# gallilmaimon/DISSC

Hardware: AMD Instinct MI355X
Metric: audio-sec/sec (RTF) HiFi-GAN resynth, 10s x32 batch (higher is better)
Workload: dtype f32

## Files before the change

dissc_amd/_lib.py:

```python
import ctypes
import os

import torch

_HERE = os.path.dirname(os.path.abspath(__file__))
_LIB_NAME = "libdissc_hip.so"


def library_path():
    return os.environ.get("DISSC_HIP_LIB") or os.path.join(_HERE, _LIB_NAME)


class DisscError(RuntimeError):
    pass


class DisscTensor(ctypes.Structure):
    _fields_ = [("name", ctypes.c_char_p), ("data", ctypes.c_void_p),
                ("shape", ctypes.c_int64 * 4), ("ndim", ctypes.c_int32)]


MAX_UPS, MAX_RK = 8, 4


class DisscGenConfig(ctypes.Structure):
    _fields_ = [("model_in_dim", ctypes.c_int32), ("upsample_initial_channel", ctypes.c_int32),
                ("num_upsamples", ctypes.c_int32), ("upsample_rates", ctypes.c_int32 * MAX_UPS),
                ("upsample_kernel_sizes", ctypes.c_int32 * MAX_UPS), ("num_kernels", ctypes.c_int32),
                ("resblock_kernel_sizes", ctypes.c_int32 * MAX_RK),
                ("resblock_dilations", (ctypes.c_int32 * 3) * MAX_RK),
                ("num_embeddings", ctypes.c_int32), ("embedding_dim", ctypes.c_int32),
                ("num_speakers", ctypes.c_int32), ("has_f0", ctypes.c_int32), ("has_spkr", ctypes.c_int32)]


class DisscConvLaunch(ctypes.Structure):
    _fields_ = [(n, ctypes.c_int32) for n in ("family", "cfg", "bm", "bn", "rows", "p0", "np", "ntap", "pad_left")]


class DisscBf3Info(ctypes.Structure):
    _fields_ = [(n, ctypes.c_int32) for n in ("bm", "bn", "small_grid", "tile", "cols", "h4", "pad")]


class DisscWino8Plan(ctypes.Structure):
    _fields_ = [(n, ctypes.c_int32) for n in ("mi", "ni", "wps", "r", "ns", "unit", "ot", "cpr", "gx", "gy")]


def _load():
    path = library_path()
    if not os.path.exists(path):
        raise DisscError(
            f"{path} not found: build the HIP library first "
            "(python -c 'import __graft_entry__ as g; g.build()').  "
            "dissc_amd has no CPU fallback.")
    L = ctypes.CDLL(path)
    vp, i32, i64p = ctypes.c_void_p, ctypes.c_int, ctypes.c_void_p
    L.dissc_last_error.restype = ctypes.c_char_p
    L.dissc_abi_version.restype = i32
    L.dissc_device_count.restype = i32
    L.dissc_device_name.argtypes = [i32, ctypes.c_char_p, ctypes.c_size_t]
    L.dissc_gen_create.argtypes = [ctypes.POINTER(DisscGenConfig), ctypes.POINTER(DisscTensor),
                                   ctypes.c_size_t, ctypes.POINTER(vp)]
    L.dissc_gen_create_ex.argtypes = [ctypes.POINTER(DisscGenConfig), ctypes.POINTER(DisscTensor),
                                      ctypes.c_size_t, i32, ctypes.POINTER(vp)]
    L.dissc_gen_destroy.argtypes = [vp]
    L.dissc_gen_destroy.restype = None
    L.dissc_gen_hop.argtypes = [vp]
    L.dissc_gen_workspace_bytes.argtypes = [vp, i32, i32]
    L.dissc_gen_workspace_bytes.restype = ctypes.c_size_t
    L.dissc_gen_flops.argtypes = [vp, ctypes.c_int64]
    L.dissc_gen_flops.restype = ctypes.c_double
    L.dissc_gen_flops_executed.argtypes = [vp, ctypes.c_int64]
    L.dissc_gen_flops_executed.restype = ctypes.c_double
    L.dissc_gen_forward.argtypes = [vp, i64p, vp, i64p, vp, i32, i32, vp, vp, ctypes.c_size_t, vp]
    L.dissc_conv1d.argtypes = [vp, vp, vp, vp, vp, i32, i32, i32, i32, i32, i32, i32, i32,
                               ctypes.c_float, vp]
    L.dissc_conv_transpose1d.argtypes = [vp, vp, vp, vp, vp, i32, i32, i32, i32, i32, i32, i32, i32,
                                         ctypes.c_float, vp]
    L.dissc_conv1d_prec.argtypes = [vp, vp, vp, vp, vp, i32, i32, i32, i32, i32, i32, i32, i32, ctypes.c_float, i32, vp]
    L.dissc_conv_transpose1d_prec.argtypes = [vp, vp, vp, vp, vp, i32, i32, i32, i32, i32, i32, i32, i32, ctypes.c_float, i32, vp]
    L.dissc_pred_create.argtypes = [i32, ctypes.POINTER(DisscTensor), ctypes.c_size_t, ctypes.POINTER(vp)]
    L.dissc_pred_destroy.argtypes = [vp]
    L.dissc_pred_destroy.restype = None
    L.dissc_pred_workspace_bytes.argtypes = [vp, i32, i32]
    L.dissc_pred_workspace_bytes.restype = ctypes.c_size_t
    L.dissc_len_set_norm.argtypes = [vp, ctypes.c_float, ctypes.c_float]
    L.dissc_len_forward.argtypes = [vp, vp, vp, vp, i32, i32, vp, i32, vp, ctypes.c_size_t, vp]
    L.dissc_pitch_forward.argtypes = [vp, vp, vp, vp, i32, i32, i32, vp, vp, i32, vp, i32, vp,
                                      ctypes.c_size_t, vp]
    L.dissc_dedup.argtypes = [vp, vp, i32, i32, vp, vp, vp, vp]
    L.dissc_len_carryover.argtypes = [vp, vp, i32, i32, vp, vp, vp]
    L.dissc_expand.argtypes = [vp, vp, vp, i32, i32, vp, i32, vp]
    L.dissc_hubert_create.argtypes = [i32, ctypes.POINTER(DisscTensor), ctypes.c_size_t, vp, i32,
                                      ctypes.POINTER(vp)]
    L.dissc_hubert_create_ex.argtypes = [i32, ctypes.POINTER(DisscTensor), ctypes.c_size_t, vp, i32, i32,
                                         ctypes.POINTER(vp)]
    L.dissc_hubert_precision.argtypes = [vp]
    L.dissc_hubert_destroy.argtypes = [vp]
    L.dissc_hubert_destroy.restype = None
    L.dissc_hubert_frames.argtypes = [i32]
    L.dissc_hubert_workspace_bytes.argtypes = [vp, i32, i32]
    L.dissc_hubert_workspace_bytes.restype = ctypes.c_size_t
    L.dissc_hubert_forward.argtypes = [vp, vp, vp, i32, i32, vp, vp, vp, ctypes.c_size_t, vp]
    L.dissc_kmeans_assign.argtypes = [vp, vp, vp, i32, i32, i32, vp, vp]
    L.dissc_mfma_peak.argtypes = [i32, ctypes.POINTER(ctypes.c_float)]
    L.dissc_erf_check.argtypes = [vp, vp, i32, vp]
    L.dissc_attention.argtypes = [vp, vp, i32, i32, i32, i32, vp, vp]
    L.dissc_layernorm_cf.argtypes = [vp, vp, vp, vp, i32, i32, i32, ctypes.c_float, vp, vp]
    L.dissc_set_option.argtypes = [ctypes.c_char_p, i32]
    L.dissc_get_option.argtypes = [ctypes.c_char_p, ctypes.POINTER(ctypes.c_int)]
    L.dissc_conv_bench.argtypes = [i32] * 9 + [ctypes.POINTER(ctypes.c_float)]
    L.dissc_conv1d_s2.argtypes = [vp, vp, vp, vp, vp] + [i32] * 9 + [vp]
    L.dissc_conv1d_s2_prec.argtypes = [vp, vp, vp, vp, vp] + [i32] * 9 + [vp]
    L.dissc_linear_prec.argtypes = [vp, vp, vp, vp, vp, vp] + [i32] * 7 + [vp]
    L.dissc_conv_s2_bench.argtypes = [i32] * 5 + [ctypes.POINTER(ctypes.c_float)]
    L.dissc_pair_bench.argtypes = [i32] * 8 + [ctypes.POINTER(ctypes.c_float)]
    L.dissc_pair_info.argtypes = [i32] * 3 + [ctypes.POINTER(ctypes.c_int)] * 2
    L.dissc_conv_info.argtypes = [i32] * 7 + [ctypes.POINTER(DisscConvLaunch), i32, ctypes.POINTER(ctypes.c_int)]
    L.dissc_wino8_info.argtypes = [i32] * 6 + [ctypes.POINTER(DisscWino8Plan)]
    L.dissc_resblock1d_bf3.argtypes = [vp, vp, vp, vp, vp, i32, i32, i32, vp, i32, i32, ctypes.c_float, i32, ctypes.c_float, i32, i32, vp]
    L.dissc_bf3_info.argtypes = [i32] * 6 + [vp, i32, i32, ctypes.POINTER(DisscBf3Info)]
    L.dissc_respair1d.argtypes = [vp] * 8 + [i32] * 6 + [ctypes.c_float, i32, ctypes.c_float, i32, vp]
    L.dissc_wav_postprocess.argtypes = [vp, vp, i32, i32, vp]
    L.dissc_pitch_stats.argtypes = [vp, vp, i32, vp, vp, vp, vp]
    i64 = ctypes.c_longlong
    L.dissc_pack_rows.argtypes = [vp, i64, vp, vp, i32, i32, vp, vp]
    L.dissc_comm_unique_id.argtypes = [ctypes.c_char_p]
# ... 76 lines not shown
```

dissc_amd/csrc/common.h:

```cpp
#pragma once
#include <hip/hip_runtime.h>
#include <stdint.h>
#include <stdio.h>

#include <atomic>
#include <functional>
#include <mutex>
#include <string>
#include <vector>

#include "../../include/dissc_hip.h"

#ifndef DISSC_EXPERIMENTAL
#define DISSC_EXPERIMENTAL 0
#endif

namespace dissc {

void set_error(const char* fmt, ...);

#define DISSC_OPTION_LIST_DEFAULT(X) \
  X(multistream, 1, "multistream") \
  X(pair_dma, 1, "pair_dma") \
  X(precision, 0, "precision") \
  X(enc_precision, 0, "enc_precision") \
  X(use_mfma32, 1, "mfma32") \
  X(ragged_enum, 1, "ragged_enum") \
  X(lin128, 1, "lin128") \
  X(conv2s128, 1, "conv2s128") \
  X(xcd_order, 11, "xcd_order") \
  X(xcd_mg, 0, "xcd_mg") \
  X(small_grid, 1, "small_grid") \
  X(kernel_dbg, 0, "kernel_dbg") \
  X(wino_sv, 1, "wino_sv") \
  X(wino8_c64_wide, 3, "wino8_c64_wide") \
  X(wino8_mask, 0450770550, "wino8_mask") \
  X(wino8_r4_mask, 0770770010, "wino8_r4_mask") \
  X(wino8_r4, 1, "wino8_r4") \
  X(wino8, 1, "wino8") \
  X(wino, 1, "wino") \
  X(hubert_split, 1, "hubert_split") \
  X(pair_max_c, 32, "pair_max_c") \
  X(pair_f23, 3, "pair_f23") \
  X(pair_tc6, 3, "pair_tc6") \
  X(pair_f23_c64, 1, "pair_f23_c64") \
  X(pair_tc6_c64, 1, "pair_tc6_c64")
#define DISSC_OPTION_LIST_EXPERIMENTAL(X) \
  X(graphs, 0, "graphs") \
  X(graph_frames, 2048, "graph_frames") \
  X(enc_tc, 0, "enc_tc") \
  X(s2tc_xmode, 0, "s2tc_xmode") \
  X(pair_wino, 0, "pair_wino") \
  X(pairw_chv, 2, "pairw_chv")
#if DISSC_EXPERIMENTAL
#define DISSC_OPTION_LIST(X) DISSC_OPTION_LIST_DEFAULT(X) DISSC_OPTION_LIST_EXPERIMENTAL(X)
#else
#define DISSC_OPTION_LIST(X) DISSC_OPTION_LIST_DEFAULT(X)
#endif
struct Options {
#define DISSC_OPT_FIELD(f, d, k) int f = d;
  DISSC_OPTION_LIST(DISSC_OPT_FIELD)
#undef DISSC_OPT_FIELD
#if !DISSC_EXPERIMENTAL
#define DISSC_OPT_CONST(f, d, k) static constexpr int f = d;
  DISSC_OPTION_LIST_EXPERIMENTAL(DISSC_OPT_CONST)
#undef DISSC_OPT_CONST
#endif
  int cfg_for_bm[5] = {6, 5, 7, 1, 0};
  int cfg32_for_bm[4] = {3, 2, 1, 0};
};
extern Options g_defaults;
extern thread_local const Options* t_opts;
inline const Options& opts() { return t_opts ? *t_opts : g_defaults; }
extern int g_graph_hits, g_graph_captures;
struct OptScope {
  const Options* prev;
  explicit OptScope(const Options* o) : prev(t_opts) { t_opts = o; }
  ~OptScope() { t_opts = prev; }
  OptScope(const OptScope&) = delete;
  OptScope& operator=(const OptScope&) = delete;
};

extern thread_local int g_conv_prec;
struct PrecScope {
  const int prev;
  explicit PrecScope(int p) : prev(g_conv_prec) { g_conv_prec = p; }
  ~PrecScope() { g_conv_prec = prev; }
  PrecScope(const PrecScope&) = delete;
  PrecScope& operator=(const PrecScope&) = delete;
};

#define DISSC_HIP_CHECK(expr)                                                       \
  do {                                                                              \
    hipError_t _e = (expr);                                                         \
    if (_e != hipSuccess) {                                                         \
      dissc::set_error("%s failed: %s (%s:%d)", #expr, hipGetErrorString(_e),       \
                       __FILE__, __LINE__);                                         \
      return DISSC_EHIP;                                                            \
    }                                                                               \
// ... 222 lines not shown
struct DevPairW {
  float* w1 = nullptr;
  float* w2 = nullptr;
  float* b1 = nullptr;
  float* b2 = nullptr;
  int C = 0, KS = 0, dil = 1;
  int form = 0;
};
bool pair_f23_supported(int C, int KS, int dil);
bool pair_tc6_supported(int C, int KS, int dil);
bool pairw43_built();
int pack_pairw43(const float* w, int C, int KS, float** dev);
int launch_pairw43(const DevPairW& pw, const float* x, float* out, const Batch& bt, const EpiSpec& ep, int ld, float slope,
                   hipStream_t stream);
bool pairw_supported(int C, int KS, int dil);
bool pair_form_supported(int form, int C, int KS, int dil);
int pair_reg_tile(int form, int C, int KS, int dil);
int make_pairw(const float* w1, const float* b1, const float* w2, const float* b2, int C, int KS, int dil, int form, DevPairW& pw);
void free_pairw(DevPairW& pw);
int launch_respair_wino(const DevPairW& pw, const float* x, float* out, const Batch& bt, const EpiSpec& ep, int ld, float slope,
                        hipStream_t stream);

bool respair_supported(int C, int KS, int dil);
int launch_respair(const DevConv& c1, const DevConv& c2, const float* x, float* out, const Batch& bt, const EpiSpec& ep, int ld,
                   float slope, hipStream_t stream);

bool resblock_bf3_supported(int C, int KS, const int* dil);
void pack_resblock_bf3(int C, int KS, const float* const* w6, std::vector<float>& packed);
struct Bf3Block { int C, KS; const int* dil; const float *wpack, *bias; };
int launch_resblock_bf3(const Bf3Block& blk, const float* x, const Batch& bt, const EpiSpec& ep, int ld, float slope, int m0, int m1,
                        hipStream_t stream);
struct ResblockBf3Plan { int NW, NI, COLS, PAD, H4, BN; };
int resblock_bf3_plan(int C, int KS, const int* dil, int m0, int m1, ResblockBf3Plan& p);

struct DevS2tc {
  float* wpack = nullptr;
  float* bias = nullptr;
  int CIN = 0, M = 0, act = 0;
};
bool s2tc_supported(int Cout, int Cin, int KS, int stride);
int make_s2tc(const float* w, const float* bias, int Cout, int Cin, DevS2tc& dc);
void free_s2tc(DevS2tc& dc);
double s2tc_executed_macs_per_out(int Cout, int Cin);
int run_s2tc(const DevS2tc& dc, const float* x, float* out, const Batch& bt, int ldx, int ldo, hipStream_t stream);

struct ZeroSpans {
  float* p[DISSC_MAX_RK];
  int n;
};
void launch_embed_concat(const int64_t* code, const float* f0, const int64_t* spkr,
                         const float* dict_w, const float* spkr_w, const int32_t* lengths, int B,
                         int T, int E, int has_f0, int has_spkr, int n_codes, int n_spk, float* x,
                         int ldx, const ZeroSpans& zs, hipStream_t stream);
void launch_conv_post(const float* x, const float* w, const float* bias, const int32_t* lengths,
                      int len_mul, int B, int C, int KS, int L, int ldx, long long x_bstride,
                      float slope, float* wav, int ldw, hipStream_t stream);
void launch_wav_postprocess(float* wav, const int32_t* n_samples, int B, int ld,
                            hipStream_t stream);

}
```

dissc_amd/csrc/gen_misc.hip:

```cpp
#include "common.h"

namespace dissc {

__global__ void embed_concat_kernel(const int64_t* __restrict__ code, const float* __restrict__ f0,
                                    const int64_t* __restrict__ spkr,
                                    const float* __restrict__ dict_w,
                                    const float* __restrict__ spkr_w,
                                    const int32_t* __restrict__ lengths, int T, int E, int has_f0,
                                    int has_spkr, int n_codes, int n_spk, float* __restrict__ x,
                                    int ldx, int C, const ZeroSpans zs) {
  const int b = blockIdx.z;
  const int c = blockIdx.y;
  const int t = blockIdx.x * blockDim.x + threadIdx.x;
  if (blockIdx.x == 0 && c == 0 && b == 0 && threadIdx.x < ZERO_TAIL)
    for (int j = 0; j < zs.n; ++j) zs.p[j][threadIdx.x] = 0.f;
  const int len = lengths ? lengths[b] : T;
  if (t >= len) return;
  float v;
  if (c < E) {
    long long id = code[(size_t)b * T + t];
    id = id < 0 ? 0 : (id >= n_codes ? n_codes - 1 : id);
    v = dict_w[(size_t)id * E + c];
  } else if (has_f0 && c == E) {
    v = f0[(size_t)b * T + t];
  } else {
    long long id = spkr[b];
    id = id < 0 ? 0 : (id >= n_spk ? n_spk - 1 : id);
    v = spkr_w[(size_t)id * E + (c - E - (has_f0 ? 1 : 0))];
  }
  x[((size_t)b * C + c) * ldx + t] = v;
}

void launch_embed_concat(const int64_t* code, const float* f0, const int64_t* spkr,
                         const float* dict_w, const float* spkr_w, const int32_t* lengths, int B,
                         int T, int E, int has_f0, int has_spkr, int n_codes, int n_spk, float* x,
                         int ldx, const ZeroSpans& zs, hipStream_t stream) {
  const int C = E + (has_f0 ? 1 : 0) + (has_spkr ? E : 0);
  dim3 grid((T + 127) / 128, C, B);
  hipLaunchKernelGGL(embed_concat_kernel, grid, dim3(128), 0, stream, code, f0, spkr, dict_w,
                     spkr_w, lengths, T, E, has_f0, has_spkr, n_codes, n_spk, x, ldx, C, zs);
}

constexpr int POST_TILE = 512;
__global__ void __launch_bounds__(256) conv_post_kernel(const float* __restrict__ x,
                                                        const float* __restrict__ w,
                                                        const float* __restrict__ bias,
                                                        const int32_t* __restrict__ lengths,
                                                        int len_mul, int C, int KS, int L, int ldx,
                                                        long long x_bstride, float slope,
                                                        float* __restrict__ wav, int ldw) {
  extern __shared__ float xs[];
  const int b = blockIdx.y;
  const int len = lengths ? lengths[b] * len_mul : L;
  const int t0 = blockIdx.x * POST_TILE;
  float* wb = wav + (size_t)b * ldw;
  if (t0 >= len) {
    for (int i = threadIdx.x; i < POST_TILE; i += 256)
      if (t0 + i < L) wb[t0 + i] = 0.f;
    return;
  }
  const int halo = KS / 2;
  const int W = POST_TILE + KS - 1;
  const float* xb = x + (size_t)b * x_bstride;
  for (int e = threadIdx.x; e < C * W; e += 256) {
    const int ci = e / W, u = e - ci * W;
    const int t = t0 - halo + u;
    float v = 0.f;
    if (t >= 0 && t < len) {
      v = xb[(size_t)ci * ldx + t];
      v = v > 0.f ? v : v * slope;
    }
    xs[e] = v;
  }
  __syncthreads();
  const float bz = bias[0];
#pragma unroll
  for (int i = 0; i < POST_TILE / 256; ++i) {
    const int u = threadIdx.x + i * 256;
    const int t = t0 + u;
    if (t >= L) continue;
    float s = bz;
    for (int ci = 0; ci < C; ++ci)
      for (int j = 0; j < KS; ++j) s = fmaf(w[ci * KS + j], xs[ci * W + u + j], s);
    wb[t] = t < len ? tanhf(s) : 0.f;
  }
}

__global__ void __launch_bounds__(256) conv_post7_kernel(const float* __restrict__ x, const float* __restrict__ w,
                                                         const float* __restrict__ bias,
                                                         const int32_t* __restrict__ lengths, int len_mul, int C,
                                                         int L, int ldx, long long x_bstride, float slope,
                                                         float* __restrict__ wav, int ldw) {
  const int b = blockIdx.y;
// ... 221 lines not shown
```

dissc_amd/csrc/generator.hip:

```cpp
#include <algorithm>
#include <functional>
#include <map>
#include <mutex>
#include <string>
#include <tuple>
#include <vector>

#include "gen_plan.h"

using namespace dissc;


static hipStream_t shared_aux_stream(int chain, int prio) {
  static std::mutex mu;
  static std::map<std::tuple<int, int, int>, hipStream_t> pool;
  int dev = 0;
  if (hipGetDevice(&dev) != hipSuccess) return nullptr;
  std::lock_guard<std::mutex> lock(mu);
  auto key = std::make_tuple(dev, chain, prio);
  auto it = pool.find(key);
  if (it != pool.end()) return it->second;
  hipStream_t st = nullptr;
  if (hipStreamCreateWithPriority(&st, hipStreamNonBlocking, prio) != hipSuccess) return nullptr;
  pool[key] = st;
  return st;
}

struct dissc_gen {
  Options opt;
  DisscGenConfig cfg;
  int hop = 1;
  DevConv conv_pre;
  std::vector<std::vector<DevConv>> ups;
  std::vector<ChainPlan> plan;
  std::vector<DevConv> rb1, rb2;
  std::vector<DevPairW> pw;
  std::vector<float*> fused_w, fused_b;
  float* post_w = nullptr;
  float* post_b = nullptr;
  int post_C = 0, post_KS = 0;
  float* dict_w = nullptr;
  float* spkr_w = nullptr;
  std::vector<int> stage_C, stage_mul;
  hipStream_t aux[DISSC_MAX_RK] = {nullptr, nullptr, nullptr, nullptr};
  hipEvent_t ev_x = nullptr, ev_fin[DISSC_MAX_RK] = {nullptr, nullptr, nullptr, nullptr};
  struct GraphEntry {
    const void *code, *f0, *spkr, *lengths, *out, *ws;
    int B, T;
    hipGraphExec_t exec;
    unsigned long long stamp;
  };
  std::vector<GraphEntry> graphs;
  hipStream_t cap_stream = nullptr;
  unsigned long long graph_clock = 0;
  int graph_failures = 0;
  ~dissc_gen() {
    for (auto& e : graphs) (void)hipGraphExecDestroy(e.exec);
    if (cap_stream) (void)hipStreamDestroy(cap_stream);
    free_conv(conv_pre);
    for (auto& v : ups) for (auto& c : v) free_conv(c);
    for (auto& c : rb1) free_conv(c);
    for (auto& c : rb2) free_conv(c);
    for (auto& c : pw) free_pairw(c);
    for (float* p : fused_w) if (p) (void)hipFree(p);
    for (float* p : fused_b) if (p) (void)hipFree(p);
    if (post_w) (void)hipFree(post_w);
    if (post_b) (void)hipFree(post_b);
    for (int j = 0; j < DISSC_MAX_RK; ++j)
      if (ev_fin[j]) (void)hipEventDestroy(ev_fin[j]);
    if (ev_x) (void)hipEventDestroy(ev_x);
    if (dict_w) (void)hipFree(dict_w);
    if (spkr_w) (void)hipFree(spkr_w);
  }
};

static inline size_t round_up(size_t x, size_t m) { return (x + m - 1) / m * m; }

extern "C" {

int dissc_gen_create(const DisscGenConfig* cfg, const DisscTensor* weights, size_t n_weights,
                     dissc_gen_t* out) {
  return dissc_gen_create_ex(cfg, weights, n_weights, -1, out);
}

int dissc_gen_create_ex(const DisscGenConfig* cfg, const DisscTensor* weights, size_t n_weights, int precision,
                        dissc_gen_t* out) {
  if (precision < -1 || precision > 1) {
    set_error("dissc_gen_create_ex: precision %d (use -1 = process option, 0 = fp32, 1 = split-bf16)", precision);
    return DISSC_EINVAL;
  }
  const int prec = precision < 0 ? g_defaults.precision : precision;
  if (!cfg || !weights || !out) {
    set_error("dissc_gen_create: null argument");
    return DISSC_EINVAL;
  }
  if (cfg->num_upsamples < 1 || cfg->num_upsamples > DISSC_MAX_UPS || cfg->num_kernels < 1 ||
      cfg->num_kernels > DISSC_MAX_RK) {
    set_error("dissc_gen_create: unsupported num_upsamples=%d / num_kernels=%d", cfg->num_upsamples,
              cfg->num_kernels);
    return DISSC_EINVAL;
  }
  std::map<std::string, const DisscTensor*> byname;
  for (size_t i = 0; i < n_weights; ++i) byname[weights[i].name] = &weights[i];
  auto get = [&](const std::string& name, std::initializer_list<int64_t> shape,
                 const float** p) -> int {
    auto it = byname.find(name);
    if (it == byname.end()) {
      set_error("dissc_gen_create: missing tensor '%s'", name.c_str());
      return DISSC_ENOTFOUND;
    }
    const DisscTensor* t = it->second;
    size_t d = 0;
    bool ok = (size_t)t->ndim == shape.size();
    for (int64_t s : shape) {
      if (ok && t->shape[d] != s) ok = false;
      ++d;
    }
    if (!ok) {
      set_error("dissc_gen_create: tensor '%s' has the wrong shape", name.c_str());
      return DISSC_EINVAL;
    }
    *p = t->data;
    return DISSC_OK;
  };

  dissc_gen* g = new dissc_gen();
  g->opt = g_defaults;
  g->opt.precision = prec;
  OptScope opt_scope(&g->opt);
  g->cfg = *cfg;
  PrecScope prec_scope(prec);
  int rc = DISSC_OK;
  const float *w = nullptr, *b = nullptr;
  const int c0 = cfg->upsample_initial_channel;
  const int in_dim = cfg->model_in_dim;
  const int E = cfg->embedding_dim;
  auto fail = [&](int code) {
    delete g;
    return code;
  };
  std::vector<std::function<int()>> tasks;
  if (in_dim != E + (cfg->has_f0 ? 1 : 0) + (cfg->has_spkr ? E : 0)) {
    set_error("dissc_gen_create: model_in_dim %d != embedding_dim %d (+1 f0) (+%d spkr)", in_dim, E, E);
    return fail(DISSC_EINVAL);
  }
  if ((rc = get("conv_pre.weight", {c0, in_dim, 7}, &w))) return fail(rc);
  if ((rc = get("conv_pre.bias", {c0}, &b))) return fail(rc);
  tasks.push_back([=]() { return make_conv(w, b, c0, in_dim, 7, 1, g->conv_pre); });

  int ch = c0, mul = 1;
  g->ups.resize(cfg->num_upsamples);
  const int nk = cfg->num_kernels;
  g->plan.resize((size_t)cfg->num_upsamples * nk);
  g->rb1.resize((size_t)cfg->num_upsamples * nk * 3);
  g->rb2.resize((size_t)cfg->num_upsamples * nk * 3);
  g->pw.resize((size_t)cfg->num_upsamples * nk * 3);
  g->fused_w.assign((size_t)cfg->num_upsamples * nk, nullptr);
  g->fused_b.assign((size_t)cfg->num_upsamples * nk, nullptr);
  for (int i = 0; i < cfg->num_upsamples; ++i) {
    const int s = cfg->upsample_rates[i], k = cfg->upsample_kernel_sizes[i];
    if (s < 1 || k < s || (k - s) % 2 != 0) {
      set_error("dissc_gen_create: upsample k=%d s=%d unsupported", k, s);
      return fail(DISSC_EINVAL);
    }
    const int cout = ch / 2;
    char name[96];
    snprintf(name, sizeof(name), "ups.%d.weight", i);
    if ((rc = get(name, {ch, cout, k}, &w))) return fail(rc);
    snprintf(name, sizeof(name), "ups.%d.bias", i);
    if ((rc = get(name, {cout}, &b))) return fail(rc);
    tasks.push_back([=]() { return make_convT(w, b, ch, cout, k, s, g->ups[i]); });
    ch = cout;
    mul *= s;
    g->stage_C.push_back(ch);
    g->stage_mul.push_back(mul);
    for (int j = 0; j < nk; ++j) {
      const int rk = cfg->resblock_kernel_sizes[j];
      if (rk % 2 != 1) {
        set_error("dissc_gen_create: even resblock kernel size %d unsupported", rk);
        return fail(DISSC_EINVAL);
      }
      const int* dl = cfg->resblock_dilations[j];
      const size_t cj = (size_t)i * nk + j;
      const ChainPlan& cp = g->plan[cj] = plan_chain(ch, rk, dl, prec);
      const float* w6[6];
      const float* b6[6];
      for (int l = 0; l < 6; ++l) {
        snprintf(name, sizeof(name), "resblocks.%d.convs%d.%d.weight", (int)cj, 1 + l % 2, l / 2);
        if ((rc = get(name, {ch, ch, rk}, &w6[l]))) return fail(rc);
        snprintf(name, sizeof(name), "resblocks.%d.convs%d.%d.bias", (int)cj, 1 + l % 2, l / 2);
        if ((rc = get(name, {ch}, &b6[l]))) return fail(rc);
      }
      if (cp.form != ChainForm::pairs) {
        std::vector<float> fw, fb;
        pack_resblock_bf3(ch, rk, w6, fw);
        for (const float* bl : b6) fb.insert(fb.end(), bl, bl + ch);
        if ((rc = upload(fw, &g->fused_w[cj]))) return fail(rc);
        if ((rc = upload(fb, &g->fused_b[cj]))) return fail(rc);
        continue;
      }
      for (int m = 0; m < 3; ++m) {
        const PairPlan p = cp.pair[m];
        const size_t idx = cj * 3 + m;
        const int d = dl[m];
        const float *w1 = w6[2 * m], *b1 = b6[2 * m], *w2 = w6[2 * m + 1], *b2 = b6[2 * m + 1];
        if (p.form == PairForm::fused_td) {
          tasks.push_back([=]() { return make_pairw(w1, b1, w2, b2, ch, rk, d, p.reg_form, g->pw[idx]); });
        } else {
          tasks.push_back([=]() { return make_pair_conv(p.conv[0], w1, b1, ch, rk, d, g->rb1[idx]); });
          tasks.push_back([=]() { return make_pair_conv(p.conv[1], w2, b2, ch, rk, 1, g->rb2[idx]); });
        }
      }
    }
  }
  g->hop = mul;
  if ((rc = get("conv_post.weight", {1, ch, 7}, &w))) return fail(rc);
  if ((rc = get("conv_post.bias", {1}, &b))) return fail(rc);
  g->post_C = ch;
  g->post_KS = 7;
  if ((rc = upload(std::vector<float>(w, w + ch * 7), &g->post_w))) return fail(rc);
  if ((rc = upload(std::vector<float>(b, b + 1), &g->post_b))) return fail(rc);
  if ((rc = get("dict.weight", {cfg->num_embeddings, E}, &w))) return fail(rc);
  if ((rc = upload(std::vector<float>(w, w + (size_t)cfg->num_embeddings * E), &g->dict_w)))
    return fail(rc);
  if (cfg->has_spkr) {
    if ((rc = get("spkr.weight", {cfg->num_speakers, E}, &w))) return fail(rc);
    if ((rc = upload(std::vector<float>(w, w + (size_t)cfg->num_speakers * E), &g->spkr_w)))
      return fail(rc);
  }
  if ((rc = run_pack_tasks(tasks, pack_thread_count(), g->opt, prec))) return fail(rc);
  if (opts().multistream && nk > 1) {
    if (hipEventCreateWithFlags(&g->ev_x, hipEventDisableTiming) != hipSuccess) return fail(DISSC_EHIP);
    for (int j = 0; j < nk; ++j) {
      if (hipEventCreateWithFlags(&g->ev_fin[j], hipEventDisableTiming) != hipSuccess) return fail(DISSC_EHIP);
      int lo = 0, hi = 0;
      (void)hipDeviceGetStreamPriorityRange(&lo, &hi);
      const int prio = lo + (hi - lo) * j / (nk - 1);
      if (j > 0 && !(g->aux[j] = shared_aux_stream(j, prio))) return fail(DISSC_EHIP);
    }
  }
  *out = g;
  return DISSC_OK;
}

void dissc_gen_destroy(dissc_gen_t g) { delete g; }

int dissc_gen_hop(dissc_gen_t g) { return g ? g->hop : 0; }

constexpr size_t BUF_GUARD = 64;
static size_t gen_buf_floats(const dissc_gen* g, int B, int Tmax) {
  size_t per = (size_t)g->cfg.upsample_initial_channel * round_up(Tmax + ZERO_TAIL, 4);
  per = std::max(per, (size_t)g->cfg.model_in_dim * round_up(Tmax + ZERO_TAIL, 4));
  for (size_t i = 0; i < g->stage_C.size(); ++i)
    per = std::max(per, (size_t)g->stage_C[i] * round_up((size_t)Tmax * g->stage_mul[i] + ZERO_TAIL, 4));
  return round_up(per * B + BUF_GUARD + 512, 64);
}

size_t dissc_gen_workspace_bytes(dissc_gen_t g, int B, int Tmax) {
  if (!g || B <= 0 || Tmax <= 0) return 0;
  OptScope opt_scope(&g->opt);
  return (size_t)(2 + 2 * g->cfg.num_kernels) * gen_buf_floats(g, B, Tmax) * sizeof(float) + 256;
}

static double gen_macs(const dissc_gen* g, bool executed) {
  double macs = g->conv_pre.macs_per_t;
  int mul = 1;
  const int nk = g->cfg.num_kernels;
  for (int i = 0; i < g->cfg.num_upsamples; ++i) {
    for (auto& c : g->ups[i]) macs += c.macs_per_t * mul;
    mul = g->stage_mul[i];
    for (int j = 0; j < nk; ++j)
      for (const PairPlan& p : g->plan[(size_t)i * nk + j].pair)
        macs += pair_macs(p, g->stage_C[i], g->cfg.resblock_kernel_sizes[j], executed) * mul;
  }
  macs += (double)g->post_C * g->post_KS * mul;
  return macs;
}

double dissc_gen_flops(dissc_gen_t g, int64_t frames) { return g ? 2.0 * gen_macs(g, false) * (double)frames : 0; }

double dissc_gen_flops_executed(dissc_gen_t g, int64_t frames) { return g ? 2.0 * gen_macs(g, true) * (double)frames : 0; }

static int gen_forward_body(dissc_gen_t g, const int64_t* code, const float* f0, const int64_t* spkr,
                            const int32_t* lengths, int B, int Tmax, float* wav_out, void* workspace,
                            hipStream_t stream);

int dissc_gen_forward(dissc_gen_t g, const int64_t* code, const float* f0, const int64_t* spkr,
                      const int32_t* lengths, int B, int Tmax, float* wav_out, void* workspace,
                      size_t workspace_bytes, void* stream_) {
  if (!g || !code || !wav_out || !workspace || (g->cfg.has_f0 && !f0) ||
      (g->cfg.has_spkr && !spkr)) {
    set_error("dissc_gen_forward: null argument");
    return DISSC_EINVAL;
  }
  OptScope opt_scope(&g->opt);
  if (B <= 0 || Tmax <= 0) {
    set_error("dissc_gen_forward: B=%d Tmax=%d", B, Tmax);
    return DISSC_EINVAL;
  }
  if ((long long)Tmax * g->hop > 2000000000LL) {
    set_error("dissc_gen_forward: Tmax=%d too long", Tmax);
    return DISSC_EINVAL;
  }
  if (workspace_bytes < dissc_gen_workspace_bytes(g, B, Tmax)) {
    set_error("dissc_gen_forward: workspace %zu < %zu bytes", workspace_bytes,
              dissc_gen_workspace_bytes(g, B, Tmax));
    return DISSC_ENOMEM;
  }
  hipStream_t stream = (hipStream_t)stream_;
#if !DISSC_EXPERIMENTAL
  return gen_forward_body(g, code, f0, spkr, lengths, B, Tmax, wav_out, workspace, stream);
#else
  if (!opts().graphs || g->graph_failures >= 2 || (long long)B * Tmax > opts().graph_frames)
    return gen_forward_body(g, code, f0, spkr, lengths, B, Tmax, wav_out, workspace, stream);
  for (auto& e : g->graphs)
    if (e.code == code && e.f0 == f0 && e.spkr == spkr && e.lengths == lengths && e.out == wav_out && e.ws == workspace &&
        e.B == B && e.T == Tmax) {
      e.stamp = ++g->graph_clock;
      ++g_graph_hits;
      DISSC_HIP_CHECK(hipGraphLaunch(e.exec, stream));
      return DISSC_OK;
    }
  if (!g->cap_stream && hipStreamCreateWithFlags(&g->cap_stream, hipStreamNonBlocking) != hipSuccess) {
    (void)hipGetLastError();
    return gen_forward_body(g, code, f0, spkr, lengths, B, Tmax, wav_out, workspace, stream);
  }
  hipGraph_t graph = nullptr;
  hipGraphExec_t exec = nullptr;
  int rc = DISSC_EHIP;
  if (hipStreamBeginCapture(g->cap_stream, hipStreamCaptureModeThreadLocal) == hipSuccess) {
    rc = gen_forward_body(g, code, f0, spkr, lengths, B, Tmax, wav_out, workspace, g->cap_stream);
    const hipError_t e = hipStreamEndCapture(g->cap_stream, &graph);
    if (rc == DISSC_OK && (e != hipSuccess || !graph)) rc = DISSC_EHIP;
    if (rc == DISSC_OK && hipGraphInstantiate(&exec, graph, nullptr, nullptr, 0) != hipSuccess) rc = DISSC_EHIP;
    if (graph) (void)hipGraphDestroy(graph);
  }
  if (rc != DISSC_OK) {
    (void)hipGetLastError();
    ++g->graph_failures;
    return gen_forward_body(g, code, f0, spkr, lengths, B, Tmax, wav_out, workspace, stream);
  }
  if (g->graphs.size() >= 8) {
    size_t old = 0;
    for (size_t i = 1; i < g->graphs.size(); ++i)
      if (g->graphs[i].stamp < g->graphs[old].stamp) old = i;
    (void)hipGraphExecDestroy(g->graphs[old].exec);
    g->graphs.erase(g->graphs.begin() + old);
  }
  ++g_graph_captures;
  g->graphs.push_back({code, f0, spkr, lengths, wav_out, workspace, B, Tmax, exec, ++g->graph_clock});
  DISSC_HIP_CHECK(hipGraphLaunch(exec, stream));
  return DISSC_OK;
#endif
}

static int gen_forward_body(dissc_gen_t g, const int64_t* code, const float* f0, const int64_t* spkr,
                            const int32_t* lengths, int B, int Tmax, float* wav_out, void* workspace,
                            hipStream_t stream) {
  const size_t nbuf = gen_buf_floats(g, B, Tmax);
  float* base = (float*)round_up((size_t)workspace, 256);
  float* X = base;
  float* ACC = base + nbuf;
  float* TMPj[DISSC_MAX_RK];
  float* XKj[DISSC_MAX_RK];
  ZeroSpans zs;
  for (int j = 0; j < g->cfg.num_kernels; ++j) {
    TMPj[j] = base + (size_t)(2 + 2 * j) * nbuf + BUF_GUARD;
    XKj[j] = base + (size_t)(3 + 2 * j) * nbuf;
    zs.p[j] = TMPj[j] - ZERO_TAIL;
  }
  zs.n = g->cfg.num_kernels;
  float* TMP = TMPj[0];
  const bool multi = g->ev_x != nullptr;
  const DisscGenConfig& c = g->cfg;
  int rc;

  const int ld0 = (int)round_up(Tmax, 4);
  launch_embed_concat(code, f0, spkr, g->dict_w, g->spkr_w, lengths, B, Tmax, c.embedding_dim,
                      c.has_f0, c.has_spkr, c.num_embeddings, c.num_speakers, TMP, ld0, zs, stream);
  Batch bt = batch_of(lengths, 1, B, Tmax);
  if ((rc = run_conv(g->conv_pre, TMP, ACC, bt, EpiSpec(), c.model_in_dim, ld0, ld0, 1.0f, stream))) return rc;
  int ch = c.upsample_initial_channel, mul = 1, ld = ld0;
  const int nk = c.num_kernels;
  for (int i = 0; i < c.num_upsamples; ++i) {
    const int s = c.upsample_rates[i];
    const int ch_out = ch / 2, mul_out = mul * s;
    const int ld_out = (int)round_up((size_t)Tmax * mul_out, 4);
    const int ngrp = (int)g->ups[i].size();
    const bool par_ups = multi && ngrp > 1 && ngrp <= nk;
    if (par_ups) DISSC_HIP_CHECK(hipEventRecord(g->ev_x, stream));
    for (int gi = 0; gi < ngrp; ++gi) {
      hipStream_t sg = (par_ups && gi > 0) ? g->aux[gi] : stream;
      if (par_ups && gi > 0) DISSC_HIP_CHECK(hipStreamWaitEvent(sg, g->ev_x, 0));
      if ((rc = run_conv(g->ups[i][gi], ACC, X, bt, EpiSpec(), ch, ld, ld_out, 0.1f, sg))) return rc;
      if (par_ups && gi > 0) {
        DISSC_HIP_CHECK(hipEventRecord(g->ev_fin[gi], sg));
        DISSC_HIP_CHECK(hipStreamWaitEvent(stream, g->ev_fin[gi], 0));
      }
    }
    ch = ch_out; mul = mul_out; ld = ld_out;
    bt = batch_of(lengths, mul, B, Tmax * mul);
    if (multi) DISSC_HIP_CHECK(hipEventRecord(g->ev_x, stream));
    for (int j = 0; j < nk; ++j) {
      hipStream_t sj = (multi && j > 0) ? g->aux[j] : stream;
      if (multi && j > 0) DISSC_HIP_CHECK(hipStreamWaitEvent(sj, g->ev_x, 0));
      const size_t cj = (size_t)i * nk + j;
      const ChainPlan& cp = g->plan[cj];
      const int rk = c.resblock_kernel_sizes[j];
      const int* dl = c.resblock_dilations[j];
      Bf3Block bf3;
      bf3.C = ch; bf3.KS = rk; bf3.dil = dl; bf3.wpack = g->fused_w[cj]; bf3.bias = g->fused_b[cj];
      float* TMPc = multi ? TMPj[j] : TMPj[0];
      float* XKc = multi ? XKj[j] : XKj[0];
      const EpiSpec mrf = epi_of(mrf_epi(j, nk), nullptr, ACC, (float)nk);
      auto acc_turn = [&]() -> int {
        if (multi && j > 0) DISSC_HIP_CHECK(hipStreamWaitEvent(sj, g->ev_fin[j - 1], 0));
        return DISSC_OK;
      };
      if (cp.form == ChainForm::bf3_block) {
        if ((rc = acc_turn()) || (rc = launch_resblock_bf3(bf3, X, bt, mrf, ld, 0.1f, 0, 3, sj))) return rc;
        if (multi) DISSC_HIP_CHECK(hipEventRecord(g->ev_fin[j], sj));
        continue;
      }
      const float* x = X;
      for (int m = 0; m < 3; ++m) {
        const size_t idx = cj * 3 + m;
        const bool last = m == 2;
        float* nxt = x == XKc ? TMPc : XKc;
        const PairForm pf = cp.pair[m].form;
        if (cp.form == ChainForm::bf3_pairs) {
          if (last && (rc = acc_turn())) return rc;
          rc = launch_resblock_bf3(bf3, x, bt, last ? mrf : epi_of(EPI_STORE, nullptr, nxt), ld, 0.1f, m, m + 1, sj);
          x = nxt;
        } else if (pf == PairForm::fused || pf == PairForm::fused_td) {
// ... 41 lines not shown
```

include/dissc_hip.h:

```cpp
#ifndef DISSC_HIP_H
#define DISSC_HIP_H

#include <stddef.h>
#include <stdint.h>

#ifdef __cplusplus
extern "C" {
#endif

#define DISSC_OK 0
#define DISSC_EINVAL (-1)
#define DISSC_ENOMEM (-2)
#define DISSC_EHIP (-3)
#define DISSC_ENOTFOUND (-4)
#define DISSC_ENOTSUP (-5)
#define DISSC_ECOMM (-6)

typedef struct {
  const char* name;
  const float* data;
  int64_t shape[4];
  int32_t ndim;
} DisscTensor;

const char* dissc_last_error(void);
int dissc_abi_version(void);
int dissc_device_count(void);
int dissc_device_name(int dev, char* buf, size_t buflen);

#define DISSC_MAX_UPS 8
#define DISSC_MAX_RK 4

typedef struct {
  int32_t model_in_dim;
  int32_t upsample_initial_channel;
  int32_t num_upsamples;
  int32_t upsample_rates[DISSC_MAX_UPS];
  int32_t upsample_kernel_sizes[DISSC_MAX_UPS];
  int32_t num_kernels;
  int32_t resblock_kernel_sizes[DISSC_MAX_RK];
  int32_t resblock_dilations[DISSC_MAX_RK][3];
  int32_t num_embeddings;
  int32_t embedding_dim;
  int32_t num_speakers;
  int32_t has_f0;
  int32_t has_spkr;
} DisscGenConfig;

typedef struct dissc_gen* dissc_gen_t;

int dissc_gen_create(const DisscGenConfig* cfg, const DisscTensor* weights, size_t n_weights,
                     dissc_gen_t* out);
int dissc_gen_create_ex(const DisscGenConfig* cfg, const DisscTensor* weights, size_t n_weights, int precision,
                        dissc_gen_t* out);
void dissc_gen_destroy(dissc_gen_t g);
int dissc_gen_hop(dissc_gen_t g);
size_t dissc_gen_workspace_bytes(dissc_gen_t g, int B, int Tmax);
double dissc_gen_flops(dissc_gen_t g, int64_t frames);
double dissc_gen_flops_executed(dissc_gen_t g, int64_t frames);
int dissc_gen_forward(dissc_gen_t g, const int64_t* code, const float* f0, const int64_t* spkr,
                      const int32_t* lengths, int B, int Tmax, float* wav_out, void* workspace,
                      size_t workspace_bytes, void* stream);
int dissc_conv1d(const float* x, const float* w_host, const float* bias_host, float* y,
                 const int32_t* lengths, int B, int Cin, int Cout, int k, int dilation, int ldx,
                 int ldo, int Lmax, float in_slope, void* stream);
int dissc_conv_transpose1d(const float* x, const float* w_host, const float* bias_host, float* y,
                           const int32_t* lengths, int B, int Cin, int Cout, int k, int stride,
                           int ldx, int ldo, int Lmax, float in_slope, void* stream);
int dissc_conv1d_prec(const float* x, const float* w_host, const float* bias_host, float* y,
                      const int32_t* lengths, int B, int Cin, int Cout, int k, int dilation, int ldx,
                      int ldo, int Lmax, float in_slope, int prec, void* stream);
int dissc_conv_transpose1d_prec(const float* x, const float* w_host, const float* bias_host, float* y,
                                const int32_t* lengths, int B, int Cin, int Cout, int k, int stride,
                                int ldx, int ldo, int Lmax, float in_slope, int prec, void* stream);

int dissc_conv1d_s2(const float* x, const float* w_host, const float* bias_host, float* y, const int32_t* lengths_in, int B,
                    int Cin, int Cout, int k, int ldx, int ldo, int Lmax_in, int act, int form, void* stream);
int dissc_conv1d_s2_prec(const float* x, const float* w_host, const float* bias_host, float* y, const int32_t* lengths_in, int B,
                         int Cin, int Cout, int k, int ldx, int ldo, int Lmax_in, int act, int prec, void* stream);
int dissc_linear_prec(const float* x, const float* w_host, const float* bias_host, const float* res, float* y,
                      const int32_t* lengths, int B, int Cin, int Cout, int ld, int Tmax, int act, int prec, void* stream);
int dissc_conv_s2_bench(int B, int C, int L, int form, int iters, float* ms_out);

int dissc_set_option(const char* key, int value);
int dissc_get_option(const char* key, int* value);

int dissc_conv_bench(int B, int Cin, int Cout, int k, int dilation, int L, int epi, int iters,
                     int flags, float* ms_out);

int dissc_respair1d(const float* x, const float* w1_host, const float* b1_host, const float* w2_host, const float* b2_host,
                    float* y, float* acc, const int32_t* lengths, int B, int C, int k, int dilation, int ld, int Lmax,
                    float slope, int epi, float mrf_div, int mode, void* stream);
int dissc_pair_bench(int B, int C, int k, int dilation, int L, int epi, int iters, int mode, float* ms_out);
int dissc_pair_info(int C, int k, int dilation, int* form_out, int* tile_out);
typedef struct {
  int32_t family, cfg, bm, bn, rows;
  int32_t p0, np, ntap, pad_left;
} DisscConvLaunch;
int dissc_conv_info(int Cin, int Cout, int k, int dilation, int up, int B, int Lmax_out, DisscConvLaunch* out, int max_out,
                    int* n_out);

typedef struct {
  int32_t mi, ni, wps, r, ns;
  int32_t unit, ot, cpr, gx, gy;
} DisscWino8Plan;
int dissc_wino8_info(int C, int k, int dilation, int R, int B, int Lmax, DisscWino8Plan* out);

int dissc_resblock1d_bf3(const float* x, const float* const* w6_host, const float* const* b6_host, float* acc,
                         const int32_t* lengths, int B, int C, int k, const int32_t* dil3, int ld, int Lmax, float slope,
                         int epi, float mrf_div, int m0, int m1, void* stream);
typedef struct {
  int32_t bm, bn, small_grid, tile;
  int32_t cols, h4, pad;
} DisscBf3Info;
int dissc_bf3_info(int Cout, int Cin, int k, int dilation, int B, int Lmax, const int32_t* dil3, int m0, int m1,
// ... 171 lines not shown
```

Measured before the change: 10270.

## Replace embedding concat plus conv_pre with precomputed per-code lookup tables

Since conv_pre is linear in the embedding inputs, the code precomputes at load time, per kernel tap, the product of conv_pre weights with every code embedding and every speaker embedding, plus the f0 weight column. At forward time a single kernel stages the code table in LDS and sums seven table rows per output, adding the speaker term, the f0 term and the bias, with no separate embed-concat pass and no conv_pre GEMM. The tables are built in double precision, so rounding differs slightly from the direct f32 conv. It also adds more device memory, a limit on LDS size by codebook size, and a new public pre-stage API.

Result: no change. 10360 (median of 6 runs) (+0.8%).

```diff
diff --git a/dissc_amd/_lib.py b/dissc_amd/_lib.py
--- a/dissc_amd/_lib.py
+++ b/dissc_amd/_lib.py
@@ -72,6 +72,9 @@
     L.dissc_gen_flops_executed.argtypes = [vp, ctypes.c_int64]
     L.dissc_gen_flops_executed.restype = ctypes.c_double
     L.dissc_gen_forward.argtypes = [vp, i64p, vp, i64p, vp, i32, i32, vp, vp, ctypes.c_size_t, vp]
+    if hasattr(L, "dissc_gen_pre"):
+        L.dissc_gen_pre_lut.argtypes = [vp]
+        L.dissc_gen_pre.argtypes = [vp, i64p, vp, i64p, vp, i32, i32, vp, vp, vp]
     L.dissc_conv1d.argtypes = [vp, vp, vp, vp, vp, i32, i32, i32, i32, i32, i32, i32, i32,
                                ctypes.c_float, vp]
     L.dissc_conv_transpose1d.argtypes = [vp, vp, vp, vp, vp, i32, i32, i32, i32, i32, i32, i32, i32,
diff --git a/dissc_amd/csrc/common.h b/dissc_amd/csrc/common.h
--- a/dissc_amd/csrc/common.h
+++ b/dissc_amd/csrc/common.h
@@ -44,7 +44,8 @@
   X(pair_f23, 3, "pair_f23") \
   X(pair_tc6, 3, "pair_tc6") \
   X(pair_f23_c64, 1, "pair_f23_c64") \
-  X(pair_tc6_c64, 1, "pair_tc6_c64")
+  X(pair_tc6_c64, 1, "pair_tc6_c64") \
+  X(pre_lut, 1, "pre_lut")
 #define DISSC_OPTION_LIST_EXPERIMENTAL(X) \
   X(graphs, 0, "graphs") \
   X(graph_frames, 2048, "graph_frames") \
@@ -373,6 +374,15 @@
                          const float* dict_w, const float* spkr_w, const int32_t* lengths, int B,
                          int T, int E, int has_f0, int has_spkr, int n_codes, int n_spk, float* x,
                          int ldx, const ZeroSpans& zs, hipStream_t stream);
+constexpr int PRE_KS = 7;
+constexpr size_t PRE_LUT_MAX_LDS = 64 * 1024;
+constexpr size_t PRE_LUT_MAX_BYTES = 8u << 20;
+size_t pre_lut_lds_bytes(int n_codes);
+void launch_pre_tables(const float* w_raw, const float* dict_w, const float* spkr_w, int C0, int CIN, int E, int has_f0, int n_codes,
+                       int n_spk, float* P, float* S, float* wf, hipStream_t stream);
+int launch_pre_lut(const int64_t* code, const float* f0, const int64_t* spkr, const int32_t* lengths, const float* P,
+                   const float* S, const float* wf, const float* bias, int B, int T, int C0, int n_codes, int n_spk, float* out,
+                   int ldo, const ZeroSpans& zs, hipStream_t stream);
 void launch_conv_post(const float* x, const float* w, const float* bias, const int32_t* lengths,
                       int len_mul, int B, int C, int KS, int L, int ldx, long long x_bstride,
                       float slope, float* wav, int ldw, hipStream_t stream);
diff --git a/dissc_amd/csrc/gen_misc.hip b/dissc_amd/csrc/gen_misc.hip
--- a/dissc_amd/csrc/gen_misc.hip
+++ b/dissc_amd/csrc/gen_misc.hip
@@ -1,4 +1,5 @@
 #include "common.h"
+#include "ragged_epi.h"
 
 namespace dissc {
 
@@ -39,6 +40,141 @@
   dim3 grid((T + 127) / 128, C, B);
   hipLaunchKernelGGL(embed_concat_kernel, grid, dim3(128), 0, stream, code, f0, spkr, dict_w,
                      spkr_w, lengths, T, E, has_f0, has_spkr, n_codes, n_spk, x, ldx, C, zs);
+}
+
+__global__ void __launch_bounds__(256) pre_table_kernel(const float* __restrict__ w, const float* __restrict__ emb, int rows, int E,
+                                                        int CIN, int ci0, int C0, long long s_ct, long long s_j, long long s_n,
+                                                        float* __restrict__ out) {
+  const long long i = (long long)blockIdx.x * 256 + threadIdx.x;
+  if (i >= (long long)PRE_KS * rows * C0) return;
+  const int co = (int)(i % C0);
+  const int n = (int)((i / C0) % rows);
+  const int j = (int)(i / ((long long)C0 * rows));
+  const float* wr = w + ((size_t)co * CIN + ci0) * PRE_KS + j;
+  const float* er = emb + (size_t)n * E;
+  double s = 0.0;
+  for (int ci = 0; ci < E; ++ci) s = fma((double)wr[(size_t)ci * PRE_KS], (double)er[ci], s);
+  out[(co >> 3) * s_ct + j * s_j + n * s_n + (co & 7)] = (float)s;
+}
+
+__global__ void pre_wf_kernel(const float* __restrict__ w, int CIN, int E, int has_f0, int C0, float* __restrict__ wf) {
+  const int i = blockIdx.x * 256 + threadIdx.x;
+  if (i >= PRE_KS * C0) return;
+  const int co = i % C0, j = i / C0;
+  wf[(co >> 3) * (PRE_KS * 8) + j * 8 + (co & 7)] = has_f0 ? w[((size_t)co * CIN + E) * PRE_KS + j] : 0.f;
+}
+
+void launch_pre_tables(const float* w_raw, const float* dict_w, const float* spkr_w, int C0, int CIN, int E, int has_f0, int n_codes,
+                       int n_spk, float* P, float* S, float* wf, hipStream_t stream) {
+  const long long np = (long long)PRE_KS * n_codes * C0;
+  hipLaunchKernelGGL(pre_table_kernel, dim3((unsigned)((np + 255) / 256)), dim3(256), 0, stream, w_raw, dict_w, n_codes, E, CIN, 0,
+                     C0, (long long)PRE_KS * n_codes * 8, (long long)n_codes * 8, 8LL, P);
+  if (S) {
+    const long long ns = (long long)PRE_KS * n_spk * C0;
+    hipLaunchKernelGGL(pre_table_kernel, dim3((unsigned)((ns + 255) / 256)), dim3(256), 0, stream, w_raw, spkr_w, n_spk, E, CIN,
+                       E + (has_f0 ? 1 : 0), C0, (long long)PRE_KS * 8, 8LL, (long long)C0 * PRE_KS, S);
+  }
+  hipLaunchKernelGGL(pre_wf_kernel, dim3((PRE_KS * C0 + 255) / 256), dim3(256), 0, stream, w_raw, CIN, E, has_f0, C0, wf);
+}
+
+__global__ void __launch_bounds__(256) pre_lut_kernel(const int64_t* __restrict__ code, const float* __restrict__ f0,
+                                                      const int64_t* __restrict__ spkr, const int32_t* __restrict__ lengths,
+                                                      const float* __restrict__ P, const float* __restrict__ S,
+                                                      const float* __restrict__ wf, const float* __restrict__ bias, int T, int C0,
+                                                      int n_codes, int n_spk, float* __restrict__ out, int ldo, const ZeroSpans zs) {
+  extern __shared__ float lut[];
+  const int ct = blockIdx.x, b = blockIdx.y;
+  if (ct == 0 && b == 0 && threadIdx.x < ZERO_TAIL)
+    for (int j = 0; j < zs.n; ++j) zs.p[j][threadIdx.x] = 0.f;
+  int len = lengths ? lengths[b] : T;
+  len = len < T ? len : T;
+  if (len <= 0) return;
+  const int np4 = PRE_KS * n_codes * 2;
+  float* sS = lut + np4 * 4;
+  float* sW = sS + PRE_KS * 8;
+  {
+    const f32x4* src = reinterpret_cast<const f32x4*>(P + (size_t)ct * np4 * 4);
+    f32x4* dst = reinterpret_cast<f32x4*>(lut);
+    for (int i = threadIdx.x; i < np4; i += 256) dst[i] = src[i];
+    if (threadIdx.x < PRE_KS * 8) {
+      float sv = 0.f;
+      if (S) {
+        long long id = spkr[b];
+        id = id < 0 ? 0 : (id >= n_spk ? n_spk - 1 : id);
+        sv = S[((size_t)id * (C0 >> 3) + ct) * (PRE_KS * 8) + threadIdx.x];
+      }
+      sS[threadIdx.x] = sv;
+      sW[threadIdx.x] = wf[(size_t)ct * (PRE_KS * 8) + threadIdx.x];
+    }
+  }
+  __syncthreads();
+  const int cq = threadIdx.x & 1;
+  const f32x4 bz = *reinterpret_cast<const f32x4*>(bias + ct * 8 + cq * 4);
+  const int64_t* cb = code + (size_t)b * T;
+  const float* fb = f0 ? f0 + (size_t)b * T : nullptr;
+  float* ob = out + ((size_t)b * C0 + ct * 8 + cq * 4) * ldo;
+  for (int t = 4 * (threadIdx.x >> 1); t < len; t += 512) {
+    int row[10];
+    float fv[10];
+#pragma unroll
+    for (int i = 0; i < 10; ++i) {
+      const int u = t - 3 + i;
+      row[i] = -1;
+      fv[i] = 0.f;
+      if (u >= 0 && u < len) {
+        long long id = cb[u];
+        id = id < 0 ? 0 : (id >= n_codes ? n_codes - 1 : id);
+        row[i] = (int)id * 8 + cq * 4;
+        if (fb) fv[i] = fb[u];
+      }
+    }
+    f32x4 acc[4] = {bz, bz, bz, bz};
+#pragma unroll
+    for (int j = 0; j < PRE_KS; ++j) {
+      const f32x4 sj = *reinterpret_cast<const f32x4*>(sS + j * 8 + cq * 4);
+      const f32x4 wj = *reinterpret_cast<const f32x4*>(sW + j * 8 + cq * 4);
+      const float* pj = lut + j * n_codes * 8;
+#pragma unroll
+      for (int e = 0; e < 4; ++e) {
+        if (row[e + j] < 0) continue;
+        const f32x4 p = *reinterpret_cast<const f32x4*>(pj + row[e + j]);
+#pragma unroll
+        for (int c = 0; c < 4; ++c) {
+          float s = acc[e][c] + (S ? p[c] + sj[c] : p[c]);
+          if (fb) s = fmaf(wj[c], fv[e + j], s);
+          acc[e][c] = s;
+        }
+      }
+    }
+    if (t + 4 <= len) {
+#pragma unroll
+      for (int c = 0; c < 4; ++c) {
+        const f32x4 o = {acc[0][c], acc[1][c], acc[2][c], acc[3][c]};
+        *reinterpret_cast<f32x4*>(ob + (size_t)c * ldo + t) = o;
+      }
+    } else {
+#pragma unroll
+      for (int c = 0; c < 4; ++c)
+#pragma unroll
+        for (int e = 0; e < 4; ++e)
+          if (t + e < len) ob[(size_t)c * ldo + t + e] = acc[e][c];
+    }
+  }
+}
+
+size_t pre_lut_lds_bytes(int n_codes) { return ((size_t)PRE_KS * n_codes * 8 + 2 * PRE_KS * 8) * sizeof(float); }
+
+int launch_pre_lut(const int64_t* code, const float* f0, const int64_t* spkr, const int32_t* lengths, const float* P,
+                   const float* S, const float* wf, const float* bias, int B, int T, int C0, int n_codes, int n_spk, float* out,
+                   int ldo, const ZeroSpans& zs, hipStream_t stream) {
+  if ((C0 & 7) || (ldo & 3) || misaligned16(out) || pre_lut_lds_bytes(n_codes) > PRE_LUT_MAX_LDS) {
+    set_error("launch_pre_lut: C0 = %d, ldo = %d, %d units: needs C0 %% 8 == 0, ldo %% 4 == 0, a 16-byte aligned output, <= %d B of LDS",
+              C0, ldo, n_codes, (int)PRE_LUT_MAX_LDS);
+    return DISSC_EINVAL;
+  }
+  hipLaunchKernelGGL(pre_lut_kernel, dim3(C0 / 8, B), dim3(256), pre_lut_lds_bytes(n_codes), stream, code, f0, spkr, lengths, P, S, wf, bias, T, C0,
+                     n_codes, n_spk, out, ldo, zs);
+  return DISSC_OK;
 }
 
 constexpr int POST_TILE = 512;
diff --git a/dissc_amd/csrc/generator.hip b/dissc_amd/csrc/generator.hip
--- a/dissc_amd/csrc/generator.hip
+++ b/dissc_amd/csrc/generator.hip
@@ -41,6 +41,7 @@
   int post_C = 0, post_KS = 0;
   float* dict_w = nullptr;
   float* spkr_w = nullptr;
+  float *pre_P = nullptr, *pre_S = nullptr, *pre_wf = nullptr, *pre_b = nullptr;
   std::vector<int> stage_C, stage_mul;
   hipStream_t aux[DISSC_MAX_RK] = {nullptr, nullptr, nullptr, nullptr};
   hipEvent_t ev_x = nullptr, ev_fin[DISSC_MAX_RK] = {nullptr, nullptr, nullptr, nullptr};
@@ -71,6 +72,8 @@
     if (ev_x) (void)hipEventDestroy(ev_x);
     if (dict_w) (void)hipFree(dict_w);
     if (spkr_w) (void)hipFree(spkr_w);
+    for (float* p : {pre_P, pre_S, pre_wf, pre_b})
+      if (p) (void)hipFree(p);
   }
 };
 
@@ -146,6 +149,7 @@
   }
   if ((rc = get("conv_pre.weight", {c0, in_dim, 7}, &w))) return fail(rc);
   if ((rc = get("conv_pre.bias", {c0}, &b))) return fail(rc);
+  const float *w_pre = w, *b_pre = b;
   tasks.push_back([=]() { return make_conv(w, b, c0, in_dim, 7, 1, g->conv_pre); });
 
   int ch = c0, mul = 1;
@@ -229,6 +233,28 @@
       return fail(rc);
   }
   if ((rc = run_pack_tasks(tasks, pack_thread_count(), g->opt, prec))) return fail(rc);
+  const size_t p_floats = (size_t)PRE_KS * cfg->num_embeddings * c0;
+  const size_t s_floats = cfg->has_spkr ? (size_t)PRE_KS * cfg->num_speakers * c0 : 0;
+  if (opts().pre_lut && c0 % 8 == 0 && pre_lut_lds_bytes(cfg->num_embeddings) <= PRE_LUT_MAX_LDS &&
+      (p_floats + s_floats) * sizeof(float) <= PRE_LUT_MAX_BYTES) {
+    float* w_raw = nullptr;
+    if ((rc = upload(std::vector<float>(w_pre, w_pre + (size_t)c0 * in_dim * PRE_KS), &w_raw))) return fail(rc);
+    rc = upload(std::vector<float>(b_pre, b_pre + c0), &g->pre_b);
+    if (!rc && hipMalloc((void**)&g->pre_P, p_floats * sizeof(float)) != hipSuccess) rc = DISSC_ENOMEM;
+    if (!rc && s_floats && hipMalloc((void**)&g->pre_S, s_floats * sizeof(float)) != hipSuccess) rc = DISSC_ENOMEM;
+    if (!rc && hipMalloc((void**)&g->pre_wf, (size_t)PRE_KS * c0 * sizeof(float)) != hipSuccess) rc = DISSC_ENOMEM;
+    if (!rc) {
+      launch_pre_tables(w_raw, g->dict_w, g->spkr_w, c0, in_dim, E, cfg->has_f0, cfg->num_embeddings, cfg->num_speakers, g->pre_P,
+                        g->pre_S, g->pre_wf, nullptr);
+      if (hipGetLastError() != hipSuccess || hipStreamSynchronize(nullptr) != hipSuccess) rc = DISSC_EHIP;
+    }
+    (void)hipFree(w_raw);
+    if (rc) {
+      if (rc == DISSC_ENOMEM) set_error("dissc_gen_create: no device memory for conv_pre's lookup tables");
+      else if (rc == DISSC_EHIP) set_error("dissc_gen_create: building conv_pre's lookup tables failed");
+      return fail(rc);
+    }
+  }
   if (opts().multistream && nk > 1) {
     if (hipEventCreateWithFlags(&g->ev_x, hipEventDisableTiming) != hipSuccess) return fail(DISSC_EHIP);
     for (int j = 0; j < nk; ++j) {
@@ -263,7 +289,7 @@
 }
 
 static double gen_macs(const dissc_gen* g, bool executed) {
-  double macs = g->conv_pre.macs_per_t;
+  double macs = executed && g->pre_P ? 0.0 : g->conv_pre.macs_per_t;
   int mul = 1;
   const int nk = g->cfg.num_kernels;
   for (int i = 0; i < g->cfg.num_upsamples; ++i) {
@@ -284,6 +310,35 @@
 static int gen_forward_body(dissc_gen_t g, const int64_t* code, const float* f0, const int64_t* spkr,
                             const int32_t* lengths, int B, int Tmax, float* wav_out, void* workspace,
                             hipStream_t stream);
+
+static int gen_pre(dissc_gen_t g, const int64_t* code, const float* f0, const int64_t* spkr, const int32_t* lengths, int B,
+                   int Tmax, float* xcat, float* y, const ZeroSpans& zs, hipStream_t stream) {
+  const DisscGenConfig& c = g->cfg;
+  const int ld0 = (int)round_up(Tmax, 4);
+  if (g->pre_P)
+    return launch_pre_lut(code, c.has_f0 ? f0 : nullptr, spkr, lengths, g->pre_P, g->pre_S, g->pre_wf, g->pre_b, B, Tmax,
+                          c.upsample_initial_channel, c.num_embeddings, c.num_speakers, y, ld0, zs, stream);
+  launch_embed_concat(code, f0, spkr, g->dict_w, g->spkr_w, lengths, B, Tmax, c.embedding_dim, c.has_f0, c.has_spkr,
+                      c.num_embeddings, c.num_speakers, xcat, ld0, zs, stream);
+  return run_conv(g->conv_pre, xcat, y, batch_of(lengths, 1, B, Tmax), EpiSpec(), c.model_in_dim, ld0, ld0, 1.0f, stream);
+}
+
+int dissc_gen_pre_lut(dissc_gen_t g) { return g && g->pre_P ? 1 : 0; }
+
+int dissc_gen_pre(dissc_gen_t g, const int64_t* code, const float* f0, const int64_t* spkr, const int32_t* lengths, int B,
+                  int Tmax, float* y, float* scratch, void* stream) {
+  if (!g || !code || !y || !scratch || (g->cfg.has_f0 && !f0) || (g->cfg.has_spkr && !spkr) || B <= 0 || Tmax <= 0) {
+    set_error("dissc_gen_pre: bad argument");
+    return DISSC_EINVAL;
+  }
+  OptScope opt_scope(&g->opt);
+  ZeroSpans zs;
+  zs.n = 0;
+  const int rc = gen_pre(g, code, f0, spkr, lengths, B, Tmax, scratch, y, zs, (hipStream_t)stream);
+  if (rc) return rc;
+  DISSC_HIP_CHECK(hipGetLastError());
+  return DISSC_OK;
+}
 
 int dissc_gen_forward(dissc_gen_t g, const int64_t* code, const float* f0, const int64_t* spkr,
                       const int32_t* lengths, int B, int Tmax, float* wav_out, void* workspace,
@@ -376,10 +431,8 @@
   int rc;
 
   const int ld0 = (int)round_up(Tmax, 4);
-  launch_embed_concat(code, f0, spkr, g->dict_w, g->spkr_w, lengths, B, Tmax, c.embedding_dim,
-                      c.has_f0, c.has_spkr, c.num_embeddings, c.num_speakers, TMP, ld0, zs, stream);
+  if ((rc = gen_pre(g, code, f0, spkr, lengths, B, Tmax, TMP, ACC, zs, stream))) return rc;
   Batch bt = batch_of(lengths, 1, B, Tmax);
-  if ((rc = run_conv(g->conv_pre, TMP, ACC, bt, EpiSpec(), c.model_in_dim, ld0, ld0, 1.0f, stream))) return rc;
   int ch = c.upsample_initial_channel, mul = 1, ld = ld0;
   const int nk = c.num_kernels;
   for (int i = 0; i < c.num_upsamples; ++i) {
diff --git a/include/dissc_hip.h b/include/dissc_hip.h
--- a/include/dissc_hip.h
+++ b/include/dissc_hip.h
@@ -61,6 +61,9 @@
 int dissc_gen_forward(dissc_gen_t g, const int64_t* code, const float* f0, const int64_t* spkr,
                       const int32_t* lengths, int B, int Tmax, float* wav_out, void* workspace,
                       size_t workspace_bytes, void* stream);
+int dissc_gen_pre_lut(dissc_gen_t g);
+int dissc_gen_pre(dissc_gen_t g, const int64_t* code, const float* f0, const int64_t* spkr, const int32_t* lengths, int B,
+                  int Tmax, float* y, float* scratch, void* stream);
 int dissc_conv1d(const float* x, const float* w_host, const float* bias_host, float* y,
                  const int32_t* lengths, int B, int Cin, int Cout, int k, int dilation, int ldx,
                  int ldo, int Lmax, float in_slope, void* stream);
```
